# Fannovel16/ComfyUI-Frame-Interpolation

Measured on AMD Instinct MI355X. Metric: interpolated frames/sec/GPU @1080p RIFE4.7 2x, higher is better.
Workload: dtype f32; 1 GPU; RIFE 4.7 2x, 1080x1920 synthetic frame-pair stream, 32 pairs/step/GPU resident in HBM (BASELINE.json configs[1]; SURVEY 8d config 2 clip: 33 frames torch.manual_seed(0) torch.rand); seeded random-init weights; new_frame_collective=none, launch=one process, one GPU

## Files before the change

comfyui-frame-interpolation_amd/csrc/conv_mfma.hip:

```cpp
#include "vfi_common.h"

#include <atomic>

#include <cstdlib>
#include <map>
#include <string>
#include <cstring>

namespace vfi {

typedef float f32x16 __attribute__((ext_vector_type(16)));
typedef float f32x4 __attribute__((ext_vector_type(4)));

template <int STRIDE, int TAPS, int MT, int NT, int WM, int WN, int CK, bool GROUPED, bool EXT>
__global__ __launch_bounds__(256) void conv_mfma_kernel(const ConvArgs a) {
    static_assert(WM * WN == 4, "4 waves per workgroup");
    static_assert(!GROUPED || (WN == 4 && NT == 1 && TAPS == 4), "grouped: one 2x2 tap group per wave column");
    static_assert(TAPS == 9 || TAPS == 4 || TAPS == 1, "tap rectangle 3x3 / 2x2 / 1x1");
    constexpr int KW = TAPS == 9 ? 3 : (TAPS == 4 ? 2 : 1);
    constexpr int SUBS = WM * MT;
    constexpr int SUBX = SUBS >= 2 ? 2 : 1;
    constexpr int SUBY = SUBS / SUBX;
    constexpr int TWO = SUBX * 8, THO = SUBY * 4;
    constexpr int TWI = STRIDE * (TWO - 1) + 3;
// ... 159 lines not shown
                        v = v > 0.f ? v : v * sl;
                        if (interior || (oy0 + (r >> 2) < a.Hout && ox0 + (r & 3) < a.Wout)) ob[(r >> 2) * ystr + (r & 3) * xstr] = v;
                    }
                }
            }
        }
        return;
    }
    if (!EXT && plain && GROUPED && a.out_mode == 1 && a.act == 0 && a.beta == nullptr) {
        const int Ws = 4 * a.Wout, Hs = 4 * a.Hout;
        const int planes = a.out_planes ? a.out_planes : 2;
        const bool interior = Y0 + (SUBS / SUBX) * 4 <= a.Hout && X0 + SUBX * 8 <= a.Wout;
#pragma unroll
        for (int nt = 0; nt < NT; ++nt) {
            const int co = co0 + nt * 32 + l31;
            if (co >= a.Cout) continue;
            const float bs = a.bias[g * a.Cout_p + co];
            const int c = co >> 2;
            float* lane_base = a.out + ((size_t)(n * planes + (c >> 2)) * Hs * Ws + (size_t)(2 * (g >> 1) + ((co >> 1) & 1)) * Ws +
                                        2 * (g & 1) + (co & 1)) * 4 + (c & 3);
#pragma unroll
            for (int mt = 0; mt < MT; ++mt) {
                const int s = wm * MT + mt;
                const int sx = s % SUBX, sy = s / SUBX;
                const int oy0 = Y0 + sy * 4, ox0 = X0 + sx * 8 + 4 * half;
                float* ob = lane_base + ((size_t)(4 * oy0) * Ws + 4 * ox0) * 4;
#pragma unroll
                for (int r = 0; r < 16; ++r)
                    if (interior || (oy0 + (r >> 2) < a.Hout && ox0 + (r & 3) < a.Wout))
                        ob[((r >> 2) * 4 * Ws + (r & 3) * 4) * 4] = acc[mt][nt][r] + bs;
            }
        }
        return;
    }
#pragma unroll
    for (int nt = 0; nt < NT; ++nt) {
        const int co = co0 + nt * 32 + l31;
        const bool cok = co < a.Cout;
        const float bs = a.bias[g * a.Cout_p + co];
        const float bt = a.beta ? a.beta[co] : 1.f;
#pragma unroll
        for (int mt = 0; mt < MT; ++mt) {
            const int s = wm * MT + mt;
            const int sx = s % SUBX, sy = s / SUBX;
#pragma unroll
            for (int r = 0; r < 16; ++r) {
                const int oy = Y0 + sy * 4 + (r >> 2);
                const int ox = X0 + sx * 8 + (r & 3) + 4 * half;
                if (cok && oy < a.Hout && ox < a.Wout) {
                    const size_t p = (size_t)(n * a.Hout + oy) * a.Wout + ox;
                    float v = acc[mt][nt][r] + bs;
                    if (a.beta) v *= bt;
                    if (a.res) v += a.res[p * a.res_cs + co];
                    if (a.act == 1) v = v > 0.f ? v : v * a.slope;
                        else if (a.act == 2) v = fminf(fmaxf(v, 0.f), 1.f);
                        else if (EXT && a.act == 3) v = v > 0.f ? v : v * a.prelu[co];
                        else if (EXT && a.act == 4) v = 1.0f / (1.0f + expf(-v));
                        else if (EXT && a.act == 5) v = 0.5f * v * (1.0f + erff(v * 0.70710678118654752440f));
                        if (EXT && a.post_scale != 0.f) v = v * a.post_scale + a.post_shift;
                    if (GROUPED && a.out_mode == 1) {
                        const int Ws = 4 * a.Wout, Hs = 4 * a.Hout, c = co >> 2;
                        const int Yt = 4 * oy + 2 * (g >> 1) + ((co >> 1) & 1), Xt = 4 * ox + 2 * (g & 1) + (co & 1);
                        a.out[((size_t)(n * (a.out_planes ? a.out_planes : 2) + (c >> 2)) * Hs * Ws + (size_t)Yt * Ws + Xt) * 4 + (c & 3)] = v;
                    } else if (EXT && GROUPED && a.out_mode == 2) {
                        const size_t q2 = (size_t)(n * 2 * a.Hout + 2 * oy + (g >> 1)) * (2 * a.Wout) + 2 * ox + (g & 1);
                        a.out[q2 * a.out_cs + co] = v;
                    } else {
                        a.out[p * a.out_cs + g * a.Cout_p + co] = v;
                    }
                }
            }
        }
    }
}

static const ConvVariant kVariants[] = {
    {"s1_m2n2", 1, 9, 2, 2, 4, 1, 16, 0},
    {"s1_m2n3", 1, 9, 2, 3, 4, 1, 16, 0},
    {"s1_m1n2", 1, 9, 1, 2, 4, 1, 16, 0},
    {"s1_m1n3", 1, 9, 1, 3, 4, 1, 16, 0},
    {"s1_m1n1", 1, 9, 1, 1, 4, 1, 16, 0},
    {"s1_m2n1", 1, 9, 2, 1, 4, 1, 16, 0},
    {"s1_m1n1w22", 1, 9, 1, 1, 2, 2, 16, 0},
    {"s1_m2n2w22", 1, 9, 2, 2, 2, 2, 16, 0},
    {"s2_m1n2", 2, 9, 1, 2, 4, 1, 8, 0},
    {"s2_m1n3", 2, 9, 1, 3, 4, 1, 8, 0},
    {"s2_m1n1", 2, 9, 1, 1, 4, 1, 8, 0},
    {"s2_m2n2", 2, 9, 2, 2, 4, 1, 8, 0},
    {"g_m4", 1, 4, 4, 1, 1, 4, 16, 1},
    {"g_m2", 1, 4, 2, 1, 1, 4, 16, 1},
};
int conv_num_variants() { return (int)(sizeof(kVariants) / sizeof(kVariants[0])); }
const ConvVariant& conv_variant(int i) { return kVariants[i]; }
const ConvVariant* conv_variant_lookup(int id) {
    if (id >= 0 && id < conv_num_variants()) return &kVariants[id];
    if (id >= kConv2Base && id < kConv2Base + conv2_num_variants()) return &conv2_variant(id - kConv2Base);
    return nullptr;
}

template <int STRIDE, int TAPS, int MT, int NT, int WM, int WN, int CK, bool GROUPED>
static int launch_t(ConvArgs a, hipStream_t s, const char* name) {
    constexpr int SUBS = WM * MT;
    constexpr int SUBX = SUBS >= 2 ? 2 : 1;
    constexpr int SUBY = SUBS / SUBX;
    a.tiles_x = cdiv(a.Wout, SUBX * 8);
    a.tiles_y = cdiv(a.Hout, SUBY * 4);
    VFI_REQUIRE(a.Cin_p % CK == 0, "conv %s: Cin_p=%d not a multiple of the K chunk %d", name, a.Cin_p, CK);
    VFI_REQUIRE(a.Cout_p % (GROUPED ? 32 : WN * NT * 32) == 0, "conv %s: Cout_p=%d not a multiple of the N tile %d",
                name, a.Cout_p, WN * NT * 32);
    dim3 grid(a.N * a.tiles_x * a.tiles_y, GROUPED ? a.Cout_p / 32 : a.Cout_p / (WN * NT * 32));
    TraceScope ts(name, s);
    if (a.pad_mode || a.act >= 3 || a.post_scale != 0.f || a.out_mode == 2)
        hipLaunchKernelGGL((conv_mfma_kernel<STRIDE, TAPS, MT, NT, WM, WN, CK, GROUPED, true>), grid, dim3(256), 0, s, a);
    else
        hipLaunchKernelGGL((conv_mfma_kernel<STRIDE, TAPS, MT, NT, WM, WN, CK, GROUPED, false>), grid, dim3(256), 0, s, a);
    VFI_CHECK_HIP(hipGetLastError());
    return 0;
}

static int n_cus_cached() {
    static std::atomic<int> n_of[kMaxDevices];
    int dev = 0;
    if (hipGetDevice(&dev) != hipSuccess || dev < 0 || dev >= kMaxDevices) return 256;
    int n = n_of[dev].load(std::memory_order_relaxed);
    if (!n) {
        hipDeviceProp_t p;
        if (hipGetDeviceProperties(&p, dev) == hipSuccess) n = p.multiProcessorCount;
        if (n <= 0) n = 256;
        n_of[dev].store(n, std::memory_order_relaxed);
    }
    return n;
}

int conv_pick_variant(const ConvArgs& a, int stride, bool grouped) {
    const long px = (long)(a.split_ok ? a.N : 8) * a.Hout * a.Wout;
    if (!grouped && stride == 1 && a.ntaps == 4 && a.tapmask) return kConv2Base + (a.Cin_p % 16 == 0 ? 28 : 26);
    if (!grouped && stride == 2 && a.ntaps == 4) return kConv2Base + (a.Cout_p % 64 == 0 ? 21 : 20);
    if (!grouped && stride == 1 && a.ntaps != 9) {
        const bool big = px * (a.Cout_p / 32) >= 256L * 4 * n_cus_cached();
        if (a.ntaps == 1 && a.Cout_p % 64 == 0 && a.Cin_p % 32 == 0)
            return kConv2Base + (a.Cin_p >= 512 && a.Cout_p % 128 == 0 ? 24 : 23);
        if (a.Cout_p % 64 == 0) return kConv2Base + (a.ntaps == 4 ? (big ? 14 : 15) : (big ? 16 : 17));
        return kConv2Base + (a.ntaps == 4 ? 19 : 18);
    }
    const long cus = n_cus_cached();
    if (grouped) {
        if (a.out_mode == 1 && px >= 250000) return kConv2Base + 11;
        return a.Cin_p % 16 == 0 ? 13 : kConv2Base + 11;
    }
    const bool n3 = a.Cout_p % 96 == 0;
    const bool n2 = a.Cout_p % 64 == 0;
    (void)cus;
    if (stride == 2) {
        if (n2) return kConv2Base + 7;
        if (n3) return kConv2Base + 9;
        return 10;
    }
    if (a.split_ok && (n2 || n3) && px <= 6000) return kConv2Base + 29;
    if (n2) {
        const long big_px = option(kOptM2n2Px);
        if (a.Cout_p == 64 || (big_px >= 0 && px >= big_px)) return kConv2Base + 0;
        return kConv2Base + 2;
    }
    if (n3) return px >= 100000 || a.Cin_p % 16 ? kConv2Base + 3 : 4;
    return a.Cin_p % 16 == 0 && px < 20000 ? 4 : kConv2Base + 13;
}

int conv_launch(const ConvArgs& a, int stride, bool grouped, int variant, hipStream_t s,
                const char* trace_name) {
    if (variant < 0 && grouped && option(kOptGroupedVariant) >= 0) variant = (int)option(kOptGroupedVariant);
    if (variant < 0 && trace_name) variant = variant_override(trace_name);
    if (variant < 0) variant = conv_pick_variant(a, stride, grouped);
    const ConvVariant* vp = conv_variant_lookup(variant);
    VFI_REQUIRE(vp, "conv: bad variant %d", variant);
    const ConvVariant& v = *vp;
    VFI_REQUIRE(v.stride == stride && (v.grouped != 0) == grouped && v.taps == a.ntaps,
                "conv: variant %s does not match stride %d grouped %d taps %d", v.name, stride, (int)grouped,
                a.ntaps);
    VFI_REQUIRE(a.out_mode != 1 || (grouped && a.Cout % 4 == 0 && a.Cout / 4 <= 4 * (a.out_planes ? a.out_planes : 2)),
                "conv: out_mode 1 is for grouped convs whose pixel-shuffled channels fit the planar4 output");
    VFI_REQUIRE(a.out_mode != 2 || grouped, "conv: out_mode 2 is for grouped convs");
    VFI_REQUIRE(a.act != 3 || a.prelu, "conv: act 3 needs per-channel slopes");
    VFI_REQUIRE(a.Cin_p % 8 == 0 && a.Cout_p % 32 == 0 && a.in_cs >= a.Cin_p && a.in_cs % 4 == 0,
                "conv: bad channel padding Cin_p=%d Cout_p=%d in_cs=%d", a.Cin_p, a.Cout_p, a.in_cs);
    VFI_REQUIRE(((uintptr_t)a.in & 15) == 0 && ((uintptr_t)a.w & 15) == 0, "conv: unaligned pointers");
    const char* nm = trace_name ? trace_name : v.name;
    if (variant >= kConv2Base) return conv2_launch(a, variant - kConv2Base, s, nm);
    switch (variant) {
        case 0: return launch_t<1, 9, 2, 2, 4, 1, 16, false>(a, s, nm);
        case 1: return launch_t<1, 9, 2, 3, 4, 1, 16, false>(a, s, nm);
        case 2: return launch_t<1, 9, 1, 2, 4, 1, 16, false>(a, s, nm);
        case 3: return launch_t<1, 9, 1, 3, 4, 1, 16, false>(a, s, nm);
        case 4: return launch_t<1, 9, 1, 1, 4, 1, 16, false>(a, s, nm);
        case 5: return launch_t<1, 9, 2, 1, 4, 1, 16, false>(a, s, nm);
        case 6: return launch_t<1, 9, 1, 1, 2, 2, 16, false>(a, s, nm);
        case 7: return launch_t<1, 9, 2, 2, 2, 2, 16, false>(a, s, nm);
        case 8: return launch_t<2, 9, 1, 2, 4, 1, 8, false>(a, s, nm);
        case 9: return launch_t<2, 9, 1, 3, 4, 1, 8, false>(a, s, nm);
        case 10: return launch_t<2, 9, 1, 1, 4, 1, 8, false>(a, s, nm);
        case 11: return launch_t<2, 9, 2, 2, 4, 1, 8, false>(a, s, nm);
        case 12: return launch_t<1, 4, 4, 1, 1, 4, 16, true>(a, s, nm);
        case 13: return launch_t<1, 4, 2, 1, 1, 4, 16, true>(a, s, nm);
    }
    return -3;
}

void conv3x3_taps(ConvArgs& a) {
    a.ntaps = 9;
    a.tap_y0 = a.tap_x0 = -1;
}
void deconv4x4_taps(ConvArgs& a) {
    a.ntaps = 4;
    a.tap_y0 = a.tap_x0 = 0;
}

void pack_conv3x3(const float* w, const float* bias, int Cout, int Cin, int Cin_p, int Cout_p,
                  std::vector<float>& wp, std::vector<float>& bp) {
    const int cin8 = Cin_p / 8;
    wp.assign((size_t)9 * cin8 * Cout_p * 8, 0.f);
    bp.assign(Cout_p, 0.f);
    for (int co = 0; co < Cout; ++co) {
        if (bias) bp[co] = bias[co];
        for (int ci = 0; ci < Cin; ++ci)
            for (int t = 0; t < 9; ++t)
                wp[(((size_t)t * cin8 + ci / 8) * Cout_p + co) * 8 + (ci & 7)] =
                    w[((size_t)co * Cin + ci) * 9 + t];
    }
}

void pack_deconv4x4(const float* w, const float* bias, int Cin, int Cout, int Cin_p, int Cout_p,
                    std::vector<float>& wp, std::vector<float>& bp) {
    const int cin8 = Cin_p / 8;
    wp.assign((size_t)4 * 4 * cin8 * Cout_p * 8, 0.f);
    bp.assign((size_t)4 * Cout_p, 0.f);
    for (int g = 0; g < 4; ++g) {
        const int py = g >> 1, px = g & 1;
        for (int co = 0; co < Cout; ++co) {
            if (bias) bp[(size_t)g * Cout_p + co] = bias[co];
            for (int t = 0; t < 4; ++t) {
                const int ky = 3 - py - 2 * (t >> 1), kx = 3 - px - 2 * (t & 1);
                for (int ci = 0; ci < Cin; ++ci)
                    wp[((((size_t)g * 4 + t) * cin8 + ci / 8) * Cout_p + co) * 8 + (ci & 7)] =
                        w[(((size_t)ci * Cout + co) * 4 + ky) * 4 + kx];
            }
        }
    }
}

__global__ void conv3x3_naive_kernel(const float* __restrict__ in, const float* __restrict__ w,
                                     const float* __restrict__ bias, const float* __restrict__ beta,
                                     float* __restrict__ out, int N, int H, int W, int Cin, int in_cs,
                                     int Cout, int stride, int Ho, int Wo, int act, float slope) {
    const long idx = (long)blockIdx.x * blockDim.x + threadIdx.x;
    const long total = (long)N * Ho * Wo * Cout;
    if (idx >= total) return;
    const int co = idx % Cout;
    long p = idx / Cout;
    const int ox = p % Wo;
    p /= Wo;
    const int oy = p % Ho;
    const int n = p / Ho;
    float acc = 0.f;
    for (int ky = 0; ky < 3; ++ky) {
        const int iy = oy * stride - 1 + ky;
        if (iy < 0 || iy >= H) continue;
        for (int kx = 0; kx < 3; ++kx) {
            const int ix = ox * stride - 1 + kx;
            if (ix < 0 || ix >= W) continue;
            const float* ip = in + ((size_t)(n * H + iy) * W + ix) * in_cs;
            const float* wp = w + (size_t)co * Cin * 9 + ky * 3 + kx;
            for (int ci = 0; ci < Cin; ++ci) acc = fmaf(ip[ci], wp[(size_t)ci * 9], acc);
        }
    }
    float v = acc + (bias ? bias[co] : 0.f);
    if (beta) v = v * beta[co] + in[((size_t)(n * H + oy) * W + ox) * in_cs + co];
    if (act == 1) v = v > 0.f ? v : v * slope;
    out[idx] = v;
}

int conv_naive_launch(const float* in, const float* w_dev, const float* bias_dev,
                      const float* beta_dev, float* out, int N, int H, int W, int Cin, int in_cs,
                      int Cout, int stride, int act, float slope, hipStream_t s) {
    const int Ho = (H + 2 - 3) / stride + 1, Wo = (W + 2 - 3) / stride + 1;
    const long total = (long)N * Ho * Wo * Cout;
    TraceScope ts("conv3x3_naive", s);
    hipLaunchKernelGGL(conv3x3_naive_kernel, dim3((unsigned)((total + 255) / 256)), dim3(256), 0, s, in,
                       w_dev, bias_dev, beta_dev, out, N, H, W, Cin, in_cs, Cout, stride, Ho, Wo, act,
                       slope);
    VFI_CHECK_HIP(hipGetLastError());
    return 0;
}

}
```

comfyui-frame-interpolation_amd/csrc/conv_mfma2.hip:

```cpp
#include "vfi_common.h"

#include <atomic>
#include <cstdlib>
#include <map>
#include <mutex>
#include <utility>

namespace vfi {

typedef float f32x16 __attribute__((ext_vector_type(16)));
typedef float f32x4 __attribute__((ext_vector_type(4)));
typedef __attribute__((address_space(3))) void* lds_ptr_t;
typedef const __attribute__((address_space(1))) void* glb_ptr_t;

template <int STRIDE, int TAPS, int MT, int NT, int WM, int WN, int CK, bool GROUPED>
struct Conv2Geom {
    static constexpr int KW = TAPS == 9 ? 3 : (TAPS == 4 ? 2 : 1);
    static constexpr int SUBS = WM * MT;
    static constexpr int SUBX = SUBS >= 16 ? 4 : (SUBS >= 2 ? 2 : 1);
    static constexpr int SUBY = SUBS / SUBX;
    static constexpr int TWO = SUBX * 8, THO = SUBY * 4;
    static constexpr int PADLO = (TAPS == 9 || GROUPED) ? 1 : 0;
    static constexpr int SPAN = (TAPS == 9 || GROUPED) ? 3 : KW;
    static constexpr int TWI = STRIDE * (TWO - 1) + SPAN;
// ... 409 lines not shown
        float* z = nullptr;
        int zn = 0;
    };
    static std::mutex mu;
    static std::map<std::pair<int, hipStream_t>, Ws> table;
    std::lock_guard<std::mutex> lock(mu);
    Ws& w = table[{dev, s}];
    if (w.n < floats) {
        w.p = nullptr, w.n = 0;
        VFI_CHECK_HIP(hipMalloc((void**)&w.p, floats * sizeof(float)));
        w.n = floats;
    }
    if (w.zn < cout_p) {
        w.z = nullptr, w.zn = 0;
        const int n = cout_p < 4096 ? 4096 : cout_p;
        VFI_CHECK_HIP(hipMalloc((void**)&w.z, n * sizeof(float)));
        VFI_CHECK_HIP(hipMemsetAsync(w.z, 0, n * sizeof(float), s));
        w.zn = n;
    }
    *ws = w.p, *zeros = w.z;
    return 0;
}

static int split_reduce(const ConvArgs& a, const float* ws, int ks, size_t slice, hipStream_t s) {
    TraceScope ts("conv_split_reduce", s);
    const long total = (long)a.N * a.Hout * a.Wout * a.Cout;
    hipLaunchKernelGGL(conv2_split_reduce_kernel, dim3((unsigned)((total + 255) / 256)), dim3(256), 0, s, a, ws, ks, (long)slice);
    VFI_CHECK_HIP(hipGetLastError());
    return 0;
}

template <int STRIDE, int TAPS, int MT, int NT, int WM, int WN, int CK, bool GROUPED, bool EXT, bool MASKED = false>
static int launch2_e(ConvArgs a, hipStream_t s, const char* name) {
    using G = Conv2Geom<STRIDE, TAPS, MT, NT, WM, WN, CK, GROUPED>;
    a.ksplit = 0, a.split_stride = 0;
    a.tiles_x = cdiv(a.Wout, G::TWO);
    a.tiles_y = cdiv(a.Hout, G::THO);
    VFI_REQUIRE(a.Cin_p % CK == 0, "conv2 %s: Cin_p=%d not a multiple of the K chunk %d", name, a.Cin_p, CK);
    VFI_REQUIRE(a.Cout_p % G::BN == 0, "conv2 %s: Cout_p=%d not a multiple of the N tile %d", name, a.Cout_p, G::BN);
    VFI_REQUIRE((long)a.Hin * a.Win * a.in_cs * 4 < 0x7fffffffL, "conv2 %s: image larger than 2 GiB", name);
    VFI_REQUIRE(!a.in_plane || a.in_plane >= a.Hin * a.Win * 4, "conv2 %s: bad plane stride", name);
    static std::atomic<int> occ_of[kMaxDevices];
    static std::atomic<int> cus_of[kMaxDevices];
    int dev = 0;
    VFI_CHECK_HIP(hipGetDevice(&dev));
    VFI_REQUIRE(dev >= 0 && dev < kMaxDevices, "conv2 %s: device index %d out of range", name, dev);
    int occ = occ_of[dev].load(std::memory_order_acquire);
    if (!occ) {
        VFI_CHECK_HIP(hipFuncSetAttribute(
            reinterpret_cast<const void*>(&conv_mfma2_kernel<STRIDE, TAPS, MT, NT, WM, WN, CK, GROUPED, EXT, MASKED>),
            hipFuncAttributeMaxDynamicSharedMemorySize, G::LDS_BYTES));
        int o = 0;
        VFI_CHECK_HIP(hipOccupancyMaxActiveBlocksPerMultiprocessor(
            &o, reinterpret_cast<const void*>(&conv_mfma2_kernel<STRIDE, TAPS, MT, NT, WM, WN, CK, GROUPED, EXT, MASKED>), 256,
            G::LDS_BYTES));
        hipDeviceProp_t p;
        VFI_CHECK_HIP(hipGetDeviceProperties(&p, dev));
        cus_of[dev].store(p.multiProcessorCount, std::memory_order_relaxed);
        occ = o < 1 ? 1 : o;
        occ_of[dev].store(occ, std::memory_order_release);
    }
    const int cus = cus_of[dev].load(std::memory_order_relaxed);
    const int T = a.N * a.tiles_x * a.tiles_y;
    const int ny = a.Cout_p / G::BN;
    int ks = 1;
    if (!GROUPED && !MASKED && a.out_mode == 0 && a.split_ok && split_enabled()) {
        const int nchunks = a.Cin_p / CK;
        const long wgs = (long)T * ny, want = 3L * cus * occ;
        const bool long_k = TAPS * nchunks >= 288, tiny = wgs * 8 <= (long)cus * occ && nchunks >= 16;
        if (wgs < (long)cus * occ && (long_k || tiny)) {
            ks = (int)((want + wgs - 1) / wgs);
            ks = ks > nchunks / 8 ? nchunks / 8 : ks;
            ks = ks > 16 ? 16 : ks;
            const int ks_traffic = TAPS * a.Cin_p / 576;
            ks = ks > ks_traffic ? ks_traffic : ks;
            ks = ks < 1 ? 1 : ks;
            const size_t slice = (size_t)a.N * a.Hout * a.Wout * a.Cout_p;
            while (ks > 1 && slice * ks * sizeof(float) > (256u << 20)) --ks;
            const int per = (nchunks + ks - 1) / ks;
            ks = (nchunks + per - 1) / per;
        }
    }
    if (ks > 1) {
        const size_t slice = (size_t)a.N * a.Hout * a.Wout * a.Cout_p;
        float *ws = nullptr, *zeros = nullptr;
        if (int rc = split_workspace(dev, s, slice * ks, a.Cout_p, &ws, &zeros)) return rc;
        ConvArgs p = a;
        p.out = ws, p.out_cs = a.Cout_p, p.bias = zeros, p.beta = nullptr, p.res = nullptr, p.res_cs = 0;
        p.act = 0, p.post_scale = 0.f, p.post_shift = 0.f, p.Cout = a.Cout_p;
        p.ksplit = ks, p.split_stride = (long)slice;
        {
            TraceScope ts(name, s);
            hipLaunchKernelGGL((conv_mfma2_kernel<STRIDE, TAPS, MT, NT, WM, WN, CK, GROUPED, EXT, MASKED>), dim3(T, ny, ks), dim3(256), G::LDS_BYTES, s, p);
            VFI_CHECK_HIP(hipGetLastError());
        }
        return split_reduce(a, ws, ks, slice, s);
    }
    int gx = (launch_cus(cus) * occ) / ny;
    if (gx < 1) gx = 1;
    if (gx > T || (long)T * ny < 4L * cus * occ) gx = T;
    if (MASKED) gx = T;
    dim3 grid(gx, ny);
    TraceScope ts(name, s);
    hipLaunchKernelGGL((conv_mfma2_kernel<STRIDE, TAPS, MT, NT, WM, WN, CK, GROUPED, EXT, MASKED>), grid, dim3(256), G::LDS_BYTES, s, a);
    VFI_CHECK_HIP(hipGetLastError());
    return 0;
}

template <int STRIDE, int TAPS, int MT, int NT, int WM, int WN, int CK>
static int launch2_masked(const ConvArgs& a, hipStream_t s, const char* name) {
    VFI_REQUIRE(a.tapmask && a.par_cout > 0 && a.par_cout % (WN * NT * 32) == 0 && a.Cout_p == 4 * a.par_cout && a.act <= 1 && !a.res && !a.beta && !a.in_plane,
                "conv2 %s: masked (up-sample x2 + 2x2) form needs 4 parity groups of a multiple of %d channels, act none / LeakyReLU", name, WN * NT * 32);
    return launch2_e<STRIDE, TAPS, MT, NT, WM, WN, CK, false, false, true>(a, s, name);
}

template <int STRIDE, int TAPS, int MT, int NT, int WM, int WN, int CK, bool GROUPED>
static int launch2_t(const ConvArgs& a, hipStream_t s, const char* name) {
    const bool ext = a.pad_mode || a.act >= 3 || a.post_scale != 0.f || a.out_mode == 2;
    return ext ? launch2_e<STRIDE, TAPS, MT, NT, WM, WN, CK, GROUPED, true>(a, s, name)
               : launch2_e<STRIDE, TAPS, MT, NT, WM, WN, CK, GROUPED, false>(a, s, name);
}

static const ConvVariant kVariants2[] = {
    {"d1_m2n2", 1, 9, 2, 2, 4, 1, 8, 0},
    {"d1_m2n3", 1, 9, 2, 3, 4, 1, 8, 0},
    {"d1_m1n2", 1, 9, 1, 2, 4, 1, 8, 0},
    {"d1_m1n3", 1, 9, 1, 3, 4, 1, 8, 0},
    {"d1_m2n2w22", 1, 9, 2, 2, 2, 2, 8, 0},
    {"d1_m4n2w22", 1, 9, 4, 2, 2, 2, 8, 0},
    {"d1_m2n2k16", 1, 9, 2, 2, 4, 1, 16, 0},
    {"d2_m1n2", 2, 9, 1, 2, 4, 1, 8, 0},
    {"d2_m2n2", 2, 9, 2, 2, 4, 1, 8, 0},
    {"d2_m1n3", 2, 9, 1, 3, 4, 1, 8, 0},
    {"d2_m2n1", 2, 9, 2, 1, 4, 1, 8, 0},
    {"dg_m4", 1, 4, 4, 1, 1, 4, 8, 1},
    {"dg_m8", 1, 4, 8, 1, 1, 4, 8, 1},
    {"d1_m2n1", 1, 9, 2, 1, 4, 1, 8, 0},
    {"d1t4_m2n2", 1, 4, 2, 2, 4, 1, 8, 0},
    {"d1t4_m1n2", 1, 4, 1, 2, 4, 1, 8, 0},
    {"d1t1_m2n2", 1, 1, 2, 2, 4, 1, 8, 0},
    {"d1t1_m1n2", 1, 1, 1, 2, 4, 1, 8, 0},
    {"d1t1_m2n1", 1, 1, 2, 1, 4, 1, 8, 0},
    {"d1t4_m2n1", 1, 4, 2, 1, 4, 1, 8, 0},
    {"d2t4_m2n1", 2, 4, 2, 1, 4, 1, 8, 0},
    {"d2t4_m1n2", 2, 4, 1, 2, 4, 1, 8, 0},
    {"d1_m4n2", 1, 9, 4, 2, 4, 1, 8, 0},
    {"d1t1_m1n2k32", 1, 1, 1, 2, 4, 1, 32, 0},
    {"d1t1_m2n2w22k32", 1, 1, 2, 2, 2, 2, 32, 0},
    {"d1t4_m2n2_up2", 1, 4, 2, 2, 4, 1, 8, 0},
    {"d1t4_m1n2_up2", 1, 4, 1, 2, 4, 1, 8, 0},
    {"d1t4_m2n2k16_up2", 1, 4, 2, 2, 4, 1, 16, 0},
    {"d1t4_m1n2k16_up2", 1, 4, 1, 2, 4, 1, 16, 0},
    {"d1_m1n1", 1, 9, 1, 1, 4, 1, 8, 0},
};
int conv2_num_variants() { return (int)(sizeof(kVariants2) / sizeof(kVariants2[0])); }
const ConvVariant& conv2_variant(int i) { return kVariants2[i]; }

int conv2_launch(const ConvArgs& a, int idx, hipStream_t s, const char* nm) {
    switch (idx) {
        case 0: return launch2_t<1, 9, 2, 2, 4, 1, 8, false>(a, s, nm);
        case 1: return launch2_t<1, 9, 2, 3, 4, 1, 8, false>(a, s, nm);
        case 2: return launch2_t<1, 9, 1, 2, 4, 1, 8, false>(a, s, nm);
        case 3: return launch2_t<1, 9, 1, 3, 4, 1, 8, false>(a, s, nm);
        case 4: return launch2_t<1, 9, 2, 2, 2, 2, 8, false>(a, s, nm);
        case 5: return launch2_t<1, 9, 4, 2, 2, 2, 8, false>(a, s, nm);
        case 6: return launch2_t<1, 9, 2, 2, 4, 1, 16, false>(a, s, nm);
        case 7: return launch2_t<2, 9, 1, 2, 4, 1, 8, false>(a, s, nm);
        case 8: return launch2_t<2, 9, 2, 2, 4, 1, 8, false>(a, s, nm);
        case 9: return launch2_t<2, 9, 1, 3, 4, 1, 8, false>(a, s, nm);
        case 10: return launch2_t<2, 9, 2, 1, 4, 1, 8, false>(a, s, nm);
        case 11: return launch2_t<1, 4, 4, 1, 1, 4, 8, true>(a, s, nm);
        case 12: return launch2_t<1, 4, 8, 1, 1, 4, 8, true>(a, s, nm);
        case 13: return launch2_t<1, 9, 2, 1, 4, 1, 8, false>(a, s, nm);
        case 14: return launch2_t<1, 4, 2, 2, 4, 1, 8, false>(a, s, nm);
        case 15: return launch2_t<1, 4, 1, 2, 4, 1, 8, false>(a, s, nm);
        case 16: return launch2_t<1, 1, 2, 2, 4, 1, 8, false>(a, s, nm);
        case 17: return launch2_t<1, 1, 1, 2, 4, 1, 8, false>(a, s, nm);
        case 18: return launch2_t<1, 1, 2, 1, 4, 1, 8, false>(a, s, nm);
        case 19: return launch2_t<1, 4, 2, 1, 4, 1, 8, false>(a, s, nm);
        case 20: return launch2_t<2, 4, 2, 1, 4, 1, 8, false>(a, s, nm);
        case 21: return launch2_t<2, 4, 1, 2, 4, 1, 8, false>(a, s, nm);
        case 22: return launch2_t<1, 9, 4, 2, 4, 1, 8, false>(a, s, nm);
        case 23: return launch2_t<1, 1, 1, 2, 4, 1, 32, false>(a, s, nm);
        case 24: return launch2_t<1, 1, 2, 2, 2, 2, 32, false>(a, s, nm);
        case 25: return launch2_masked<1, 4, 2, 2, 4, 1, 8>(a, s, nm);
        case 26: return launch2_masked<1, 4, 1, 2, 4, 1, 8>(a, s, nm);
        case 27: return launch2_masked<1, 4, 2, 2, 4, 1, 16>(a, s, nm);
        case 28: return launch2_masked<1, 4, 1, 2, 4, 1, 16>(a, s, nm);
        case 29: return launch2_t<1, 9, 1, 1, 4, 1, 8, false>(a, s, nm);
    }
    set_error("conv2: bad variant %d", idx);
    return -3;
}

}
```

comfyui-frame-interpolation_amd/csrc/util.hip:

```cpp
#include "vfi_common.h"

#include <cstdarg>
#include <cstdio>
#include <cstring>
#include <atomic>
#include <chrono>
#include <cstdlib>
#include <map>
#include <mutex>
#include <string>
#include <vector>

#include "../../include/vfi_hip.h"
#include "../../include/vfi_hip_test.h"

namespace vfi {

static thread_local char g_err[1024] = "";

void set_error(const char* fmt, ...) {
    va_list ap;
    va_start(ap, fmt);
    vsnprintf(g_err, sizeof(g_err), fmt, ap);
    va_end(ap);
}
const char* get_error() { return g_err; }

static const struct { const char* name; long dflt; } kOptTable[kOptCount] = {
    {"stage_quad", 14}, {"fuse_encode", 1}, {"fuse0a", 1}, {"m2n2_px", -1}, {"grouped_variant", -1}, {"splitk", 1},
    {"splat_atomic", 0}, {"splat_spill_cap", -1}, {"wino_xcd", 1}, {"deconv_wino", 1}, {"encode_batched", 1}, {"wino_quant", 1}, {"xcd_bands", 0}, {"m2m_fused", 1}, {"m2m_side", 0}, {"film_side", 1}, {"wino_probe", 0},
    {"sepconv_split_heads", 0}, {"sepconv_planar", 1},
};
static std::atomic<long> g_opt[kOptCount];
static std::atomic<bool> g_opt_init{false};
static std::mutex g_opt_mu;
static std::map<std::string, int> g_variant_override;
static std::atomic<int> g_variant_override_n{0};
static void opt_init() {
    if (g_opt_init.load(std::memory_order_acquire)) return;
    std::lock_guard<std::mutex> lk(g_opt_mu);
    if (g_opt_init.load(std::memory_order_relaxed)) return;
    for (int i = 0; i < kOptCount; ++i) g_opt[i].store(kOptTable[i].dflt, std::memory_order_relaxed);
    g_opt_init.store(true, std::memory_order_release);
}
long option(Option o) {
    opt_init();
    return g_opt[o].load(std::memory_order_relaxed);
}
#ifdef VFI_TEST_TAPS
int option_set(const char* name, long value) {
    opt_init();
    for (int i = 0; i < kOptCount; ++i)
        if (name && !strcmp(name, kOptTable[i].name)) {
            g_opt[i].store(value, std::memory_order_relaxed);
            return 0;
        }
    set_error("vfi_test_set_option: unknown option '%s'", name ? name : "(null)");
    return -2;
}
#endif
int variant_override(const char* trace_name) {
    if (!trace_name || !g_variant_override_n.load(std::memory_order_acquire)) return -1;
    std::lock_guard<std::mutex> lk(g_opt_mu);
    auto it = g_variant_override.find(trace_name);
    return it == g_variant_override.end() ? -1 : it->second;
}
#ifdef VFI_TEST_TAPS
static void variant_override_set(const char* spec) {
    std::lock_guard<std::mutex> lk(g_opt_mu);
    g_variant_override.clear();
    std::string str = spec ? spec : "";
    size_t pos = 0;
    while (pos < str.size()) {
        const size_t comma = str.find(',', pos), end = comma == std::string::npos ? str.size() : comma;
        const size_t eq = str.find('=', pos);
        if (eq != std::string::npos && eq < end) g_variant_override[str.substr(pos, eq - pos)] = atoi(str.c_str() + eq + 1);
        pos = end + 1;
    }
    g_variant_override_n.store((int)g_variant_override.size(), std::memory_order_release);
}
#endif

struct TraceRec {
    const char* name;
    hipEvent_t e0, e1;
};
static bool g_trace = false;
static std::vector<TraceRec> g_recs;
static std::vector<hipEvent_t> g_free_events;

static hipEvent_t get_event() {
    if (!g_free_events.empty()) {
        hipEvent_t e = g_free_events.back();
        g_free_events.pop_back();
        return e;
    }
    hipEvent_t e = nullptr;
    (void)hipEventCreate(&e);
    return e;
}

bool trace_on() { return g_trace; }
void trace_begin(const char* name, hipStream_t s) {
    TraceRec r;
    r.name = name;
    r.e0 = get_event();
    r.e1 = get_event();
    (void)hipEventRecord(r.e0, s);
    g_recs.push_back(r);
}
void trace_end(hipStream_t s) {
    if (!g_recs.empty()) (void)hipEventRecord(g_recs.back().e1, s);
}


}

using namespace vfi;

namespace vfi {
static std::mutex g_side_mu;
static std::vector<hipStream_t> g_side_idle;

static bool streams_together(hipStream_t st, hipStream_t c) {
    vfi_stream_spin(c, 1);
    vfi_stream_spin(st, 1);
    int together = 0;
    for (int r = 0; r < 3; ++r) {
        (void)hipStreamSynchronize(st);
        (void)hipStreamSynchronize(c);
        const auto t0 = std::chrono::steady_clock::now();
        vfi_stream_spin(st, 300);
        vfi_stream_spin(c, 300);
        (void)hipStreamSynchronize(st);
        (void)hipStreamSynchronize(c);
        together += std::chrono::duration<double, std::micro>(std::chrono::steady_clock::now() - t0).count() > 480.0;
    }
    return together >= 2;
}

hipStream_t stream_apart_from(hipStream_t st) {
    std::lock_guard<std::mutex> lk(g_side_mu);
    int dev = 0;
    (void)hipGetDevice(&dev);
    std::vector<hipStream_t> rejected;
    hipStream_t found = nullptr;
    for (int t = 0; t < 12 && !found; ++t) {
        hipStream_t c = nullptr;
        for (size_t i = 0; i < g_side_idle.size() && !c; ++i) {
            int d = -1;
            if (hipStreamGetDevice(g_side_idle[i], &d) == hipSuccess && d == dev) {
                c = g_side_idle[i];
                g_side_idle.erase(g_side_idle.begin() + i);
            }
        }
        if (!c && hipStreamCreateWithFlags(&c, hipStreamNonBlocking) != hipSuccess) break;
        if (streams_together(st, c)) rejected.push_back(c);
        else found = c;
    }
    if (!found && !rejected.empty()) {
        found = rejected.back();
        rejected.pop_back();
    }
    for (hipStream_t r : rejected) g_side_idle.push_back(r);
    return found;
}

void stream_give_back(hipStream_t side) {
    if (!side) return;
    (void)hipStreamSynchronize(side);
    std::lock_guard<std::mutex> lk(g_side_mu);
    g_side_idle.push_back(side);
}

__global__ void stream_spin_kernel(unsigned long long ticks) {
    const unsigned long long t0 = wall_clock64();
    while (wall_clock64() - t0 < ticks) __builtin_amdgcn_s_sleep(8);
}
}

extern "C" {

int vfi_init(int device) {
    int n = 0;
// ... 147 lines not shown
```

comfyui-frame-interpolation_amd/csrc/vfi_common.h:

```cpp
#pragma once
#include <hip/hip_runtime.h>
#include <stdint.h>
#include <string>
#include <vector>

namespace vfi {

void set_error(const char* fmt, ...);
const char* get_error();

#define VFI_CHECK_HIP(expr)                                                                   \
    do {                                                                                      \
        hipError_t _e = (expr);                                                               \
        if (_e != hipSuccess) {                                                               \
            ::vfi::set_error("%s failed: %s (%s:%d)", #expr, hipGetErrorString(_e), __FILE__, \
                             __LINE__);                                                       \
            return -1;                                                                        \
        }                                                                                     \
    } while (0)

#define VFI_REQUIRE(cond, ...)          \
    do {                                \
        if (!(cond)) {                  \
            ::vfi::set_error(__VA_ARGS__); \
            return -2;                  \
        }                               \
    } while (0)

bool trace_on();
void trace_begin(const char* name, hipStream_t s);
void trace_end(hipStream_t s);

struct TraceScope {
    hipStream_t s;
    bool on;
    TraceScope(const char* name, hipStream_t st) : s(st), on(trace_on()) {
        if (on) trace_begin(name, s);
    }
    ~TraceScope() {
        if (on) trace_end(s);
    }
};

int clock_probe_tag(const char* name);
int clock_probe_install(unsigned long long* dev_records, int capacity);
int wino_probe_read(unsigned* out32);

enum Option {
    kOptStageQuad,
    kOptFuseEncode,
    kOptFuse0a,
    kOptM2n2Px,
    kOptGroupedVariant,
    kOptSplitK,
    kOptSplatAtomic,
    kOptSplatSpillCap,
    kOptWinoXcd,
    kOptDeconvWino,
    kOptEncodeBatched,
    kOptWinoQuant,
    kOptXcdBands,
    kOptM2mFused,
    kOptM2mSide,
    kOptFilmSide,
    kOptWinoProbe,
    kOptSepconvSplitHeads,
    kOptSepconvPlanar,
    kOptCount
};
long option(Option o);
hipStream_t stream_apart_from(hipStream_t st);
void stream_give_back(hipStream_t side);
int option_set(const char* name, long value);
int variant_override(const char* trace_name);

int launch_cus(int device_cus);

int softsplat4_launch(const float* in, const float* flow, float* out, int N, int H, int W, hipStream_t s);

constexpr int kMaxDevices = 16;

__host__ __device__ __forceinline__ int pad_index(int i, int n, int mode) {
    if (mode == 2) i = i < 0 ? -i : (i >= n ? 2 * n - 2 - i : i);
    return min(max(i, 0), n - 1);
}

static inline int cdiv(int a, int b) { return (a + b - 1) / b; }
static inline int round_up(int a, int b) { return cdiv(a, b) * b; }

struct ConvArgs {
    const float* in;
    const float* w;
    const float* bias;
    const float* beta;
    const float* res;
    float* out;
    int N, Hin, Win, in_cs;
    int Hout, Wout, out_cs, res_cs;
    int Cin_p, Cout_p, Cout;
    int ntaps;
    int act;
    float slope;
    int tiles_x, tiles_y;
    int tap_y0, tap_x0;
    int in_plane;
    int out_mode;
    int out_planes;
    int pad_mode;
    const float* prelu;
    float post_scale, post_shift;
    int split_ok;
    const unsigned char* tapmask;
    int par_cout;
    int ksplit;
    long split_stride;
};

struct ConvVariant {
    const char* name;
    int stride, taps, mt, nt, wm, wn, ck, grouped;
};
constexpr int kConv2Base = 32;
int conv_num_variants();
const ConvVariant& conv_variant(int i);
int conv2_num_variants();
const ConvVariant& conv2_variant(int i);
int conv2_launch(const ConvArgs& a, int idx, hipStream_t s, const char* trace_name);
const ConvVariant* conv_variant_lookup(int id);
int conv_pick_variant(const ConvArgs& a, int stride, bool grouped);
int conv_launch(const ConvArgs& a, int stride, bool grouped, int variant, hipStream_t s,
                const char* trace_name);

void pack_conv3x3(const float* w_oihw, const float* bias, int Cout, int Cin, int Cin_p,
                  int Cout_p, std::vector<float>& wp, std::vector<float>& bp);
void pack_deconv4x4(const float* w_iohw, const float* bias, int Cin, int Cout, int Cin_p,
                    int Cout_p, std::vector<float>& wp, std::vector<float>& bp);
void conv3x3_taps(ConvArgs& a);

void pack_wino3x3(const float* w_oihw, int Cout, int Cin, const int* chan_map, int Cin_p, int Cout_p, std::vector<float>& wp);
void pack_deconv_as_conv3x3(const float* w_iohw, const float* bias, int Cin, int LO, std::vector<float>& w3, std::vector<float>& b3);
bool conv_wino_eligible(const ConvArgs& a);
int conv_wino_mode(int set);
int conv_wino_launch(const ConvArgs& a, int variant, hipStream_t s, const char* trace_name);
void deconv4x4_taps(ConvArgs& a);

int conv_naive_launch(const float* in, const float* w_oihw_dev, const float* bias_dev,
                      const float* beta_dev, float* out, int N, int H, int W, int Cin, int in_cs,
                      int Cout, int stride, int act, float slope, hipStream_t s);

}
```

Before: 866.0 frames/s.

## Add persistent double-buffered stride-2 3x3 MFMA conv kernel with resident weights

Adds a dedicated stride-2 3x3 convolution kernel that loops persistently over output tiles. It double-buffers input tiles into LDS with async buffer loads, prefetching the next tile during the last K chunk. For 8-wave workgroups it keeps all weights resident in LDS when they fit. The variant picker now routes plain stride-2 3x3 convs with Cout divisible by 64 or 96 to these kernels, aiming to hide load latency and cut repeated weight fetches. The cost is high LDS use and lower occupancy; non-plain cases fall back to the old variants, and optional timing probes exist only in test builds.

```diff
diff --git a/comfyui-frame-interpolation_amd/csrc/conv_mfma.hip b/comfyui-frame-interpolation_amd/csrc/conv_mfma.hip
--- a/comfyui-frame-interpolation_amd/csrc/conv_mfma.hip
+++ b/comfyui-frame-interpolation_amd/csrc/conv_mfma.hip
@@ -335,6 +335,10 @@
     const bool n2 = a.Cout_p % 64 == 0;
     (void)cus;
     if (stride == 2) {
+        if (!a.split_ok && a.ntaps == 9 && (n2 || n3)) {
+            const bool fits = a.Cin_p * (n2 ? 2 : 3) <= 78;
+            return kConv2Base + (fits ? 32 : 30) + (n2 ? 0 : 1);
+        }
         if (n2) return kConv2Base + 7;
         if (n3) return kConv2Base + 9;
         return 10;
diff --git a/comfyui-frame-interpolation_amd/csrc/conv_mfma2.hip b/comfyui-frame-interpolation_amd/csrc/conv_mfma2.hip
--- a/comfyui-frame-interpolation_amd/csrc/conv_mfma2.hip
+++ b/comfyui-frame-interpolation_amd/csrc/conv_mfma2.hip
@@ -585,11 +585,21 @@
     {"d1t4_m2n2k16_up2", 1, 4, 2, 2, 4, 1, 16, 0},
     {"d1t4_m1n2k16_up2", 1, 4, 1, 2, 4, 1, 16, 0},
     {"d1_m1n1", 1, 9, 1, 1, 4, 1, 8, 0},
+    {"d2w4_m1n2", 2, 9, 1, 2, 4, 1, 8, 0},
+    {"d2w4_m1n3", 2, 9, 1, 3, 4, 1, 8, 0},
+    {"d2w8_m1n2", 2, 9, 1, 2, 8, 1, 8, 0},
+    {"d2w8_m1n3", 2, 9, 1, 3, 8, 1, 8, 0},
 };
 int conv2_num_variants() { return (int)(sizeof(kVariants2) / sizeof(kVariants2[0])); }
 const ConvVariant& conv2_variant(int i) { return kVariants2[i]; }
 
 int conv2_launch(const ConvArgs& a, int idx, hipStream_t s, const char* nm) {
+    if (idx >= 30 && idx <= 33) {
+        const bool plain = !a.pad_mode && a.act < 3 && a.post_scale == 0.f && a.out_mode == 0 && !a.tapmask;
+        const int nt = idx & 1 ? 3 : 2;
+        if (!plain) idx = nt == 3 ? 9 : 7;
+        else return conv_s2_launch(a, idx >= 32 ? 8 : 4, nt, s, nm);
+    }
     switch (idx) {
         case 0: return launch2_t<1, 9, 2, 2, 4, 1, 8, false>(a, s, nm);
         case 1: return launch2_t<1, 9, 2, 3, 4, 1, 8, false>(a, s, nm);
diff --git a/comfyui-frame-interpolation_amd/csrc/conv_s2.hip b/comfyui-frame-interpolation_amd/csrc/conv_s2.hip
--- /dev/null
+++ b/comfyui-frame-interpolation_amd/csrc/conv_s2.hip
@@ -0,0 +1,395 @@
+#include "vfi_common.h"
+
+#include <atomic>
+#include <mutex>
+
+namespace vfi {
+
+typedef float f32x16 __attribute__((ext_vector_type(16)));
+typedef float f32x4 __attribute__((ext_vector_type(4)));
+typedef __attribute__((address_space(3))) void* lds_ptr_t;
+typedef const __attribute__((address_space(1))) void* glb_ptr_t;
+
+constexpr int kS2ProbeWords = 16;
+
+template <int WAVES, int NT>
+struct S2Geom {
+    static constexpr int TWO = 16, THO = (WAVES / 2) * 4;
+    static constexpr int TWI = 2 * (TWO - 1) + 3, THI = 2 * (THO - 1) + 3;
+    static constexpr int RP = 34;
+    static constexpr int NA = (THI * RP * 2 + 63) / 64;
+    static constexpr int A_FLOATS = NA * 256;
+    static constexpr int BN = NT * 32;
+    static constexpr int NB = 9 * NT;
+    static constexpr int B_FLOATS = NB * 256;
+    static constexpr int NAW = (NA + WAVES - 1) / WAVES;
+    static constexpr int NBW = (NB + WAVES - 1) / WAVES;
+    static constexpr int NPW = NAW + NBW;
+    static constexpr int PPS = (NPW + 8) / 9;
+    static constexpr int MAX_LDS = 160 * 1024;
+    static int lds_bytes(int bslots) { return (2 * A_FLOATS + bslots * B_FLOATS) * 4; }
+};
+
+template <int WAVES, int NT, bool SPREAD, int PROBE>
+__global__ __launch_bounds__(WAVES * 64) void conv_s2_kernel(const ConvArgs a, const int resident, unsigned* const probe_out) {
+#if defined(__HIP_DEVICE_COMPILE__)
+    using G = S2Geom<WAVES, NT>;
+    constexpr int TWI = G::TWI, TWO = G::TWO, THO = G::THO, BN = G::BN, CK = 8;
+
+    extern __shared__ __attribute__((aligned(16))) float smem[];
+
+    const int tid = threadIdx.x;
+    const int lane = tid & 63;
+    const int wave = __builtin_amdgcn_readfirstlane(tid >> 6);
+    const int half = lane >> 5, l31 = lane & 31;
+    const int cob = blockIdx.y * BN;
+    const int cin8 = a.Cin_p >> 3;
+
+#define S2_STAMP(COND_, V_)                                      \
+    if (PROBE != 0 && (COND_)) {                                 \
+        __builtin_amdgcn_sched_barrier(0);                       \
+        V_ = (unsigned)__builtin_amdgcn_s_memtime();             \
+        __builtin_amdgcn_sched_barrier(0);                       \
+    }
+    unsigned q[8] = {0, 0, 0, 0, 0, 0, 0, 0};
+    unsigned s_start = 0, s_tile = 0, s_clr = 0, s_top = 0, s_k0 = 0, s_k1 = 0, s_bar = 0, s_e1 = 0;
+    S2_STAMP(true, s_start);
+
+    const int tiles_per_img = a.tiles_x * a.tiles_y;
+    const int T = a.N * tiles_per_img;
+    const int pstr = a.in_plane ? 4 : a.in_cs;
+    const int qstr = a.in_plane ? a.in_plane : 4;
+    const int cadv = a.in_plane ? (CK / 4) * a.in_plane : CK;
+    const int img_floats = a.in_plane ? (a.in_cs / 4) * a.in_plane : a.Hin * a.Win * a.in_cs;
+    auto decode = [&](int tile, int& n, int& Y0, int& X0) {
+        n = tile / tiles_per_img;
+        const int trem = tile - n * tiles_per_img;
+        const int ty = trem / a.tiles_x;
+        Y0 = ty * THO;
+        X0 = (trem - ty * a.tiles_x) * TWO;
+    };
+    auto make_avoff = [&](int Y0, int X0, int(&avoff)[G::NAW]) {
+        const int iy0 = 2 * Y0 - 1, ix0 = 2 * X0 - 1;
+#pragma unroll
+        for (int i = 0; i < G::NAW; ++i) {
+            const int j = wave + WAVES * i;
+            const int idx = j * 64 + lane;
+            const int slot = idx >> 1;
+            const int py = slot / G::RP, col = slot - py * G::RP;
+            const int px = col < 17 ? 2 * col : 2 * col - 33;
+            const int q2 = (idx ^ (py >> 1)) & 1;
+            const int iy = iy0 + py, ix = ix0 + px;
+            const bool ok = py < G::THI && col < TWI && iy >= 0 && iy < a.Hin && ix >= 0 && ix < a.Win;
+            avoff[i] = ok ? ((iy * a.Win + ix) * pstr + q2 * qstr) * 4 : (int)0x80000000;
+        }
+    };
+    auto make_rsrc = [&](int n) {
+        return __builtin_amdgcn_make_buffer_rsrc((void*)(a.in + (size_t)n * img_floats), 0, img_floats * 4, 0x00020000);
+    };
+    const int tapstride = cin8 * a.Cout_p * 8;
+    const int c8stride = a.Cout_p * 8;
+    const float* wsrc[G::NBW];
+#pragma unroll
+    for (int i = 0; i < G::NBW; ++i) {
+        const int j = wave + WAVES * i;
+        const int t = j / NT, sub = j - t * NT;
+        wsrc[i] = a.w + (size_t)(t < 9 ? t : 0) * tapstride + (cob + sub * 32) * 8 + (lane >> 1) * 8 + ((lane ^ (lane >> 5)) & 1) * 4;
+    }
+    float* const bregion = smem + 2 * G::A_FLOATS;
+    auto issue_a = [&](const __amdgpu_buffer_rsrc_t& rs, int i, int vo, int sbyte, int buf) {
+        const int j = wave + WAVES * i;
+        if (G::NA % WAVES == 0 || j < G::NA)
+            __builtin_amdgcn_raw_ptr_buffer_load_lds(rs, (lds_ptr_t)(smem + buf * G::A_FLOATS + j * 256), 16, vo, sbyte, 0, 0);
+    };
+    auto issue_b = [&](int i, int chunk, int slot) {
+        const int j = wave + WAVES * i;
+        if (G::NB % WAVES == 0 || j < G::NB)
+            __builtin_amdgcn_global_load_lds((glb_ptr_t)(wsrc[i] + chunk * c8stride), (lds_ptr_t)(bregion + slot * G::B_FLOATS + j * 256), 16, 0, 0);
+    };
+
+    const int oyl = l31 >> 3;
+    const int arow = (2 * ((wave >> 1) * 4 + oyl) * G::RP + (wave & 1) * 8 + (l31 & 7)) * CK;
+    const int abase0 = arow + ((half ^ oyl) & 1) * 4, abase1 = arow + ((half ^ oyl ^ 1) & 1) * 4;
+    const int blane = l31 * 8 + ((half ^ (l31 >> 4)) & 1) * 4;
+
+    float bs[NT], bt[NT];
+#pragma unroll
+    for (int nt = 0; nt < NT; ++nt) {
+        const int co = cob + nt * 32 + l31;
+        bs[nt] = a.bias[co];
+        bt[nt] = a.beta ? a.beta[co] : 1.f;
+    }
+
+    const int nchunks = a.Cin_p / CK;
+    float* const outp = a.out;
+
+    int tile = blockIdx.x;
+    if (tile >= T) return;
+    int n, Y0, X0, avoff[G::NAW];
+    decode(tile, n, Y0, X0);
+    make_avoff(Y0, X0, avoff);
+    __amdgpu_buffer_rsrc_t rsrc = make_rsrc(n);
+    if (resident) {
+        for (int c = 0; c < nchunks; ++c)
+#pragma unroll
+            for (int i = 0; i < G::NBW; ++i) issue_b(i, c, c);
+    } else {
+#pragma unroll
+        for (int i = 0; i < G::NBW; ++i) issue_b(i, 0, 0);
+    }
+#pragma unroll
+    for (int i = 0; i < G::NAW; ++i) issue_a(rsrc, i, avoff[i], 0, 0);
+    __syncthreads();
+    int buf = 0;
+    for (;;) {
+        S2_STAMP(PROBE == 1, s_tile);
+        const int ntile = tile + gridDim.x;
+        const bool has_next = ntile < T;
+        int nn = 0, nY0 = 0, nX0 = 0, navoff[G::NAW];
+#pragma unroll
+        for (int i = 0; i < G::NAW; ++i) navoff[i] = avoff[i];
+        __amdgpu_buffer_rsrc_t nrsrc = rsrc;
+
+        f32x16 acc[NT];
+#pragma unroll
+        for (int nt = 0; nt < NT; ++nt)
+#pragma unroll
+            for (int r = 0; r < 16; ++r) acc[nt][r] = 0.f;
+        S2_STAMP(PROBE == 1, s_clr);
+        if (PROBE == 1) q[3] += s_clr - s_tile, ++q[6];
+
+        for (int k = 0; k < nchunks; ++k) {
+            S2_STAMP(PROBE != 0, s_top);
+            const bool last = k + 1 == nchunks;
+            const bool feed = !last || has_next;
+            if (last && has_next) {
+                decode(ntile, nn, nY0, nX0);
+                make_avoff(nY0, nX0, navoff);
+                nrsrc = make_rsrc(nn);
+            }
+            int vo[G::NAW];
+#pragma unroll
+            for (int i = 0; i < G::NAW; ++i) vo[i] = last ? navoff[i] : avoff[i];
+            __amdgpu_buffer_rsrc_t rs = rsrc;
+            if (last) rs = nrsrc;
+            const int nchunk = last ? 0 : k + 1;
+            const int sbyte = nchunk * cadv * 4;
+            if (!SPREAD && feed) {
+#pragma unroll
+                for (int i = 0; i < G::NAW; ++i) issue_a(rs, i, vo[i], sbyte, buf ^ 1);
+                if (!resident) {
+#pragma unroll
+                    for (int i = 0; i < G::NBW; ++i) issue_b(i, nchunk, buf ^ 1);
+                }
+            }
+            const float* pa0 = smem + buf * G::A_FLOATS + abase0;
+            const float* pa1 = smem + buf * G::A_FLOATS + abase1;
+            const float* pb = bregion + (resident ? k : buf) * G::B_FLOATS + blane;
+            S2_STAMP(PROBE != 0, s_k0);
+            f32x4 av[2], bv[2][NT];
+            unsigned d0[9], d1[9];
+            auto frag = [&](int t, f32x4& fa, f32x4(&fb)[NT]) {
+                const int ty = t / 3, tx = t % 3;
+                fa = *(const f32x4*)&(ty == 2 ? pa1 : pa0)[(ty * G::RP + (tx == 0 ? 0 : tx == 1 ? 17 : 1)) * CK];
+#pragma unroll
+                for (int nt = 0; nt < NT; ++nt) fb[nt] = *(const f32x4*)&pb[(t * BN + nt * 32) * 8];
+            };
+            frag(0, av[0], bv[0]);
+#pragma unroll
+            for (int st = 0; st < 9; ++st) {
+                __builtin_amdgcn_sched_barrier(0);
+#pragma unroll
+                for (int j = 0; j < 4; ++j) {
+#pragma unroll
+                    for (int nt = 0; nt < NT; ++nt)
+                        acc[nt] = __builtin_amdgcn_mfma_f32_32x32x2f32(av[st & 1][j], bv[st & 1][nt][j], acc[nt], 0, 0, 0);
+                    __builtin_amdgcn_sched_barrier(0);
+                    if (j == 0 && st + 1 < 9) {
+                        frag(st + 1, av[(st + 1) & 1], bv[(st + 1) & 1]);
+                        __builtin_amdgcn_sched_barrier(0);
+                    }
+                    if (SPREAD && j == 1 && st * G::PPS < G::NPW) {
+                        S2_STAMP(PROBE == 2, d0[st]);
+                        if (feed) {
+#pragma unroll
+                            for (int p = st * G::PPS; p < (st + 1) * G::PPS && p < G::NPW; ++p) {
+                                if (p < G::NAW) issue_a(rs, p, vo[p < G::NAW ? p : 0], sbyte, buf ^ 1);
+                                else if (!resident) issue_b(p - G::NAW, nchunk, buf ^ 1);
+                            }
+                        }
+                        __builtin_amdgcn_sched_barrier(0);
+                        S2_STAMP(PROBE == 2, d1[st]);
+                    }
+                }
+            }
+            S2_STAMP(PROBE != 0, s_k1);
+            __syncthreads();
+            S2_STAMP(PROBE != 0, s_bar);
+            if (PROBE != 0) {
+                q[0] += s_k0 - s_top, q[1] += s_k1 - s_k0, q[2] += s_bar - s_k1, ++q[5];
+                if (PROBE == 2 && SPREAD) {
+#pragma unroll
+                    for (int st = 0; st < 9; ++st)
+                        if (st * G::PPS < G::NPW) q[7] += d1[st] - d0[st];
+                }
+            }
+            buf ^= 1;
+        }
+
+        const bool fast = a.res == nullptr && (a.act == 0 || a.act == 1);
+        const int sx = wave & 1, sy = wave >> 1;
+        const int oy0 = Y0 + sy * 4, ox0 = X0 + sx * 8 + 4 * half;
+        if (fast) {
+            const int xstr = a.out_cs, ystr = a.Wout * a.out_cs;
+            const bool interior = Y0 + THO <= a.Hout && X0 + TWO <= a.Wout;
+            const bool unif01 = a.act == 0 || (a.act == 1 && a.slope >= 0.f && a.slope <= 1.f);
+            const float uslope = a.act == 1 ? a.slope : 1.0f;
+#pragma unroll
+            for (int nt = 0; nt < NT; ++nt) {
+                const int co = cob + nt * 32 + l31;
+                if (co < a.Cout) {
+                    float* ob = outp + ((size_t)(n * a.Hout + oy0) * a.Wout + ox0) * a.out_cs + co;
+                    if (unif01 && interior) {
+#pragma unroll
+                        for (int r = 0; r < 16; ++r) {
+                            const float v = (acc[nt][r] + bs[nt]) * bt[nt];
+                            ob[(r >> 2) * ystr + (r & 3) * xstr] = fmaxf(v, v * uslope);
+                        }
+                    } else {
+                        const float sl = a.act == 0 ? 1.0f : a.slope;
+#pragma unroll
+                        for (int r = 0; r < 16; ++r) {
+                            float v = (acc[nt][r] + bs[nt]) * bt[nt];
+                            v = v > 0.f ? v : v * sl;
+                            if (interior || (oy0 + (r >> 2) < a.Hout && ox0 + (r & 3) < a.Wout)) ob[(r >> 2) * ystr + (r & 3) * xstr] = v;
+                        }
+                    }
+                }
+            }
+        } else {
+#pragma unroll
+            for (int nt = 0; nt < NT; ++nt) {
+                const int co = cob + nt * 32 + l31;
+                const bool cok = co < a.Cout;
+                const int coc = cok ? co : a.Cout - 1;
+                float rv[16];
+                if (a.res) {
+#pragma unroll
+                    for (int r = 0; r < 16; ++r) {
+                        int ry = oy0 + (r >> 2), rx = ox0 + (r & 3);
+                        ry = ry < a.Hout ? ry : a.Hout - 1;
+                        rx = rx < a.Wout ? rx : a.Wout - 1;
+                        rv[r] = a.res[((size_t)(n * a.Hout + ry) * a.Wout + rx) * a.res_cs + coc];
+                    }
+                }
+#pragma unroll
+                for (int r = 0; r < 16; ++r) {
+                    const int py = oy0 + (r >> 2), px = ox0 + (r & 3);
+                    float v = acc[nt][r] + bs[nt];
+                    if (a.beta) v *= bt[nt];
+                    if (a.res) v += rv[r];
+                    if (a.act == 1) v = v > 0.f ? v : v * a.slope;
+                    else if (a.act == 2) v = fminf(fmaxf(v, 0.f), 1.f);
+                    if (cok && py < a.Hout && px < a.Wout) outp[((size_t)(n * a.Hout + py) * a.Wout + px) * a.out_cs + co] = v;
+                }
+            }
+        }
+        S2_STAMP(PROBE == 1, s_e1);
+        if (PROBE == 1) q[4] += s_e1 - s_bar;
+        if (!has_next) break;
+        tile = ntile;
+        n = nn;
+        Y0 = nY0;
+        X0 = nX0;
+        rsrc = nrsrc;
+#pragma unroll
+        for (int i = 0; i < G::NAW; ++i) avoff[i] = navoff[i];
+    }
+    if (PROBE != 0 && blockIdx.x == 0 && blockIdx.y == 0 && probe_out) {
+        unsigned s_end = 0;
+        S2_STAMP(true, s_end);
+        if (lane < kS2ProbeWords) {
+            unsigned v = 0;
+#pragma unroll
+            for (int i = 0; i < 8; ++i) v = lane == i ? q[i] : v;
+            v = lane == 8 ? s_end - s_start : lane == 10 ? (unsigned)PROBE : lane == 11 ? (unsigned)WAVES : v;
+            probe_out[wave * kS2ProbeWords + lane] = v;
+        }
+    }
+#undef S2_STAMP
+#endif
+}
+
+template <int WAVES, int NT, bool SPREAD, int PROBE>
+static int s2_launch_t(ConvArgs a, hipStream_t s, const char* name) {
+    using G = S2Geom<WAVES, NT>;
+    a.ksplit = 0, a.split_stride = 0;
+    a.tiles_x = cdiv(a.Wout, G::TWO);
+    a.tiles_y = cdiv(a.Hout, G::THO);
+    VFI_REQUIRE(a.Cin_p % 8 == 0, "conv_s2 %s: Cin_p=%d not a multiple of the K chunk 8", name, a.Cin_p);
+    VFI_REQUIRE(a.Cout_p % G::BN == 0, "conv_s2 %s: Cout_p=%d not a multiple of the N tile %d", name, a.Cout_p, G::BN);
+    VFI_REQUIRE((long)a.Hin * a.Win * a.in_cs * 4 < 0x7fffffffL, "conv_s2 %s: image larger than 2 GiB", name);
+    VFI_REQUIRE(!a.in_plane || a.in_plane >= a.Hin * a.Win * 4, "conv_s2 %s: bad plane stride", name);
+    VFI_REQUIRE(a.ntaps == 9 && a.tap_y0 == -1 && a.tap_x0 == -1, "conv_s2 %s: 3x3 taps from (-1, -1) only", name);
+    const int nchunks = a.Cin_p / 8;
+    const int resident = WAVES == 8 && G::lds_bytes(nchunks) <= G::MAX_LDS;
+    const int lds = G::lds_bytes(resident ? nchunks : 2);
+    VFI_REQUIRE(lds <= G::MAX_LDS, "conv_s2 %s: %d bytes of LDS", name, lds);
+    static std::atomic<int> attr_of[kMaxDevices];
+    static std::atomic<int> cus_of[kMaxDevices];
+    int dev = 0;
+    VFI_CHECK_HIP(hipGetDevice(&dev));
+    VFI_REQUIRE(dev >= 0 && dev < kMaxDevices, "conv_s2 %s: device index %d out of range", name, dev);
+    const void* fn = reinterpret_cast<const void*>(&conv_s2_kernel<WAVES, NT, SPREAD, PROBE>);
+    int occ_stream = attr_of[dev].load(std::memory_order_acquire);
+    if (!occ_stream) {
+        VFI_CHECK_HIP(hipFuncSetAttribute(fn, hipFuncAttributeMaxDynamicSharedMemorySize, WAVES == 8 ? G::MAX_LDS : G::lds_bytes(2)));
+        int o = 0;
+        VFI_CHECK_HIP(hipOccupancyMaxActiveBlocksPerMultiprocessor(&o, fn, WAVES * 64, G::lds_bytes(2)));
+        hipDeviceProp_t p;
+        VFI_CHECK_HIP(hipGetDeviceProperties(&p, dev));
+        cus_of[dev].store(p.multiProcessorCount, std::memory_order_relaxed);
+        occ_stream = (o < 1 ? 1 : o) + 1;
+        attr_of[dev].store(occ_stream, std::memory_order_release);
+    }
+    const int occ = WAVES == 8 ? 1 : occ_stream - 1;
+    const int cus = cus_of[dev].load(std::memory_order_relaxed);
+    const int T = a.N * a.tiles_x * a.tiles_y;
+    const int ny = a.Cout_p / G::BN;
+    int gx = (launch_cus(cus) * occ) / ny;
+    if (gx < 1) gx = 1;
+    if (gx > T || (long)T * ny < 4L * cus * occ) gx = T;
+    unsigned* probe_out = PROBE ? (unsigned*)(uintptr_t)option(kOptS2ProbeBuf) : nullptr;
+    TraceScope ts(name, s);
+    hipLaunchKernelGGL((conv_s2_kernel<WAVES, NT, SPREAD, PROBE>), dim3(gx, ny), dim3(WAVES * 64), lds, s, a, resident, probe_out);
+    VFI_CHECK_HIP(hipGetLastError());
+    return 0;
+}
+
+template <int WAVES, int NT>
+static int s2_launch_w(const ConvArgs& a, hipStream_t s, const char* name) {
+#ifdef VFI_TEST_TAPS
+    const long probe = option(kOptS2Probe);
+    if constexpr (WAVES == 4) {
+        if (option(kOptS2Spread) == 0) {
+            if (probe == 1) return s2_launch_t<WAVES, NT, false, 1>(a, s, name);
+            if (probe == 2) return s2_launch_t<WAVES, NT, false, 2>(a, s, name);
+            return s2_launch_t<WAVES, NT, false, 0>(a, s, name);
+        }
+    }
+    if (probe == 1) return s2_launch_t<WAVES, NT, true, 1>(a, s, name);
+    if (probe == 2) return s2_launch_t<WAVES, NT, true, 2>(a, s, name);
+#endif
+    return s2_launch_t<WAVES, NT, true, 0>(a, s, name);
+}
+
+int conv_s2_launch(const ConvArgs& a, int waves, int nt, hipStream_t s, const char* name) {
+    if (waves == 4 && nt == 2) return s2_launch_w<4, 2>(a, s, name);
+    if (waves == 4 && nt == 3) return s2_launch_w<4, 3>(a, s, name);
+    if (waves == 8 && nt == 2) return s2_launch_w<8, 2>(a, s, name);
+    if (waves == 8 && nt == 3) return s2_launch_w<8, 3>(a, s, name);
+    set_error("conv_s2: no %d-wave form with a %d-channel N tile", waves, nt * 32);
+    return -3;
+}
+
+}
diff --git a/comfyui-frame-interpolation_amd/csrc/util.hip b/comfyui-frame-interpolation_amd/csrc/util.hip
--- a/comfyui-frame-interpolation_amd/csrc/util.hip
+++ b/comfyui-frame-interpolation_amd/csrc/util.hip
@@ -29,7 +29,7 @@
 static const struct { const char* name; long dflt; } kOptTable[kOptCount] = {
     {"stage_quad", 14}, {"fuse_encode", 1}, {"fuse0a", 1}, {"m2n2_px", -1}, {"grouped_variant", -1}, {"splitk", 1},
     {"splat_atomic", 0}, {"splat_spill_cap", -1}, {"wino_xcd", 1}, {"deconv_wino", 1}, {"encode_batched", 1}, {"wino_quant", 1}, {"xcd_bands", 0}, {"m2m_fused", 1}, {"m2m_side", 0}, {"film_side", 1}, {"wino_probe", 0},
-    {"sepconv_split_heads", 0}, {"sepconv_planar", 1},
+    {"sepconv_split_heads", 0}, {"sepconv_planar", 1}, {"s2_probe", 0}, {"s2_probe_buf", 0}, {"s2_spread", 1},
 };
 static std::atomic<long> g_opt[kOptCount];
 static std::atomic<bool> g_opt_init{false};
diff --git a/comfyui-frame-interpolation_amd/csrc/vfi_common.h b/comfyui-frame-interpolation_amd/csrc/vfi_common.h
--- a/comfyui-frame-interpolation_amd/csrc/vfi_common.h
+++ b/comfyui-frame-interpolation_amd/csrc/vfi_common.h
@@ -66,6 +66,9 @@
     kOptWinoProbe,
     kOptSepconvSplitHeads,
     kOptSepconvPlanar,
+    kOptS2Probe,
+    kOptS2ProbeBuf,
+    kOptS2Spread,
     kOptCount
 };
 long option(Option o);
@@ -127,6 +130,7 @@
 const ConvVariant& conv2_variant(int i);
 int conv2_launch(const ConvArgs& a, int idx, hipStream_t s, const char* trace_name);
 const ConvVariant* conv_variant_lookup(int id);
+int conv_s2_launch(const ConvArgs& a, int waves, int nt, hipStream_t s, const char* trace_name);
 int conv_pick_variant(const ConvArgs& a, int stride, bool grouped);
 int conv_launch(const ConvArgs& a, int stride, bool grouped, int variant, hipStream_t s,
                 const char* trace_name);
```

Result: no change. 873.5 frames/s, median of 6 (+0.9%).
